# valeoai/NAF

Hardware: AMD Instinct MI355X
Metric: upsampled Mpixels/sec (NAF forward) (higher is better)
Workload: dtype bf16; 1 GPU; G1: 1x3x1024x1024 guidance, 1x768x64x64 features -> 1024x1024, window 7, per GPU; per_gpu_batch=1, global_batch=1, parallelism=batch-shard x1, scope=whole forward (conv stem + RoPE/pool + attention), weights=random-init NAF() defaults (dim 256, 4 heads), streams=2

## Files before the change

naf_amd/csrc/naf_api.hip:

```cpp
#include <stdarg.h>
#include <stdio.h>
#include <stdlib.h>
#include <string.h>

#include "naf_common.h"

static thread_local char g_err[512] = "";

void naf_set_error(const char* fmt, ...) {
    va_list ap;
    va_start(ap, fmt);
    vsnprintf(g_err, sizeof(g_err), fmt, ap);
    va_end(ap);
}

int naf_check_launch(const char* what) {
    const hipError_t e = hipGetLastError();
    if (e != hipSuccess) {
        naf_set_error("%s: %s", what, hipGetErrorString(e));
        return NAF_ERR_LAUNCH;
    }
    return NAF_OK;
}

// ... 599 lines not shown
    L.buf0 = off;  off = align256(off + px * 128 * 2);
    L.buf1 = off;  off = align256(off + px * 128 * 2);
    L.buf2 = off;  off = align256(off + px * 128 * 2);
    L.cat = off;   off = align256(off + px * 256 * 2);
    L.pooled = L.Ho != L.Hs || L.Wo != L.Ws;
    const size_t opx = (size_t)a->B * L.Ho * L.Wo;
    L.guide = L.pooled ? off : L.cat;
    if (L.pooled) off = align256(off + opx * 256 * 2);
    L.keys = off;  off = align256(off + (size_t)a->B * a->h * a->w * 256 * 2);
    L.vp = off;    off = align256(off + (size_t)a->B * a->h * a->w * a->C * 2);
    L.fused = fwd_rope_fusable(a);
    L.q = off;     off = align256(off + (L.fused ? 0 : opx * 256 * 2));
    L.idx_y = off; off = align256(off + (size_t)L.Ho * (a->ksize > 0 ? a->ksize : 1) * sizeof(int32_t));
    L.idx_x = off; off = align256(off + (size_t)L.Wo * (a->ksize > 0 ? a->ksize : 1) * sizeof(int32_t));
    L.total_one = off;
    L.buf3 = off;  off = align256(off + px * 128 * 2);
    L.total = off;
    return L;
}
int fwd_validate(const naf_forward_args* a) {
    NAF_REQUIRE(a != nullptr, "naf_forward: args is NULL");
    NAF_REQUIRE(a->image && a->features && a->out && a->tab_y && a->tab_x, "naf_forward: NULL tensor pointer");
    NAF_REQUIRE(a->B > 0 && a->H > 0 && a->W > 0 && a->h > 0 && a->w > 0 && a->C > 0 && a->heads > 0, "naf_forward: non-positive size");
    NAF_REQUIRE(a->nlayer >= 1 && a->nlayer <= NAF_MAX_STEM_LAYERS, "naf_forward: %d block layers (1..%d)", a->nlayer, NAF_MAX_STEM_LAYERS);
    NAF_REQUIRE(a->C % a->heads == 0, "naf_forward: %d feature channels not divisible by %d heads", a->C, a->heads);
    for (int br = 0; br < 2; ++br) {
        const naf_stem_branch& b = a->branch[br];
        NAF_REQUIRE(b.conv0_weight && b.conv0_bias, "naf_forward: branch %d: NULL conv0 parameters", br);
        NAF_REQUIRE((b.conv0_ksize == 1 || b.conv0_ksize == 3) && (b.ksize == 1 || b.ksize == 3), "naf_forward: branch %d: kernel sizes", br);
        for (int l = 0; l < a->nlayer; ++l)
            NAF_REQUIRE(b.gn_weight[l] && b.gn_bias[l] && b.conv_weight_packed[l] && b.conv_bias[l], "naf_forward: branch %d layer %d: NULL parameter", br, l);
    }
    return NAF_OK;
}
void fwd_xna_args(const naf_forward_args* a, const FwdLayout* L, bool fused, naf_xna_args* x) {
    char* ws = static_cast<char*>(a->workspace);
    const bool real = ws != nullptr && L != nullptr;
    const void* fake = reinterpret_cast<const void*>(0x100);
    const int Dv = a->C / a->heads;
    *x = naf_xna_args{};
    const int Ho = a->Ho > 0 ? a->Ho : a->H, Wo = a->Wo > 0 ? a->Wo : a->W;
    x->q = real ? ws + (fused ? L->guide : L->q) : fake;
    x->k_lr = real ? ws + L->keys : fake;
    x->v_lr = real ? ws + L->vp : fake;
    x->out = a->out;
    x->logits = a->logits;
    if (fused) {
        x->rope_tab_y = a->tab_y; x->rope_tab_x = a->tab_x;
        x->path = NAF_XNA_MFMA;
    } else {
        x->path = NAF_XNA_AUTO;
        x->idx_y = real ? reinterpret_cast<const int32_t*>(ws + L->idx_y) : static_cast<const int32_t*>(fake);
        x->idx_x = real ? reinterpret_cast<const int32_t*>(ws + L->idx_x) : static_cast<const int32_t*>(fake);
    }
    x->B = a->B; x->heads = a->heads; x->Ho = Ho; x->Wo = Wo; x->h = a->h; x->w = a->w;
    x->Dq = 256 / a->heads; x->Dv = Dv; x->ky = a->ksize; x->kx = a->ksize;
    x->out_dtype = a->out_dtype; x->scale = a->scale;
    const int64_t Dq = x->Dq;
    const int64_t qs[4] = {(int64_t)Ho * Wo * 256, Dq, (int64_t)Wo * 256, 256};
    const int64_t ks[4] = {(int64_t)a->h * a->w * 256, Dq, (int64_t)a->w * 256, 256};
    const int64_t vs[4] = {(int64_t)a->h * a->w * a->C, Dv, (int64_t)a->w * a->C, a->C};
    const int64_t os[4] = {(int64_t)Ho * Wo * a->C, Dv, (int64_t)Wo * a->C, a->C};
    for (int i = 0; i < 4; ++i) { x->q_stride[i] = qs[i]; x->k_stride[i] = ks[i]; x->v_stride[i] = vs[i]; x->o_stride[i] = os[i]; }
}
bool fwd_rope_fusable(const naf_forward_args* a) {
    if (a->heads_rope > 0 && a->heads_rope != a->heads) return false;
    if (a->heads <= 0 || a->C <= 0 || a->C % a->heads || 256 % a->heads) return false;
    naf_forward_args g = *a;
    g.workspace = nullptr;
    g.out = reinterpret_cast<void*>(0x100);
    g.tab_y = g.tab_x = reinterpret_cast<const float*>(0x100);
    naf_xna_args x;
    fwd_xna_args(&g, nullptr, true, &x);
    return xna_validate(&x) == NAF_OK && naf_xna_mfma_eligible(&x, nullptr, nullptr) && naf_xna_mfma_rope_ok(&x);
}
}

size_t naf_forward_workspace_bytes(const naf_forward_args* a) {
    if (a == nullptr || a->B <= 0 || a->H <= 0 || a->W <= 0 || a->h <= 0 || a->w <= 0 || a->C <= 0 || a->nlayer < 0) return 0;
    return fwd_layout(a).total;
}
size_t naf_forward_workspace_bytes_ex(const naf_forward_args* a, uint32_t flags) {
    if (a == nullptr || a->B <= 0 || a->H <= 0 || a->W <= 0 || a->h <= 0 || a->w <= 0 || a->C <= 0 || a->nlayer < 0) return 0;
    const FwdLayout L = fwd_layout(a);
    return (flags & NAF_FWD_ONE_STREAM) ? L.total_one : L.total;
}

int naf_forward_workspace_view(const naf_forward_args* a, int32_t which, size_t* offset, size_t* bytes) {
    NAF_REQUIRE(a != nullptr && offset != nullptr && bytes != nullptr, "naf_forward_workspace_view: NULL argument");
    NAF_REQUIRE(a->B > 0 && a->H > 0 && a->W > 0 && a->h > 0 && a->w > 0 && a->C > 0 && a->nlayer >= 0, "naf_forward_workspace_view: non-positive size");
    const FwdLayout L = fwd_layout(a);
    switch (which) {
        case NAF_FWD_BUF_GUIDANCE: *offset = L.guide; *bytes = (size_t)a->B * L.Ho * L.Wo * 256 * 2; return NAF_OK;
        case NAF_FWD_BUF_KEYS: *offset = L.keys; *bytes = (size_t)a->B * a->h * a->w * 256 * 2; return NAF_OK;
        case NAF_FWD_BUF_VALUES: *offset = L.vp; *bytes = (size_t)a->B * a->h * a->w * a->C * 2; return NAF_OK;
    }
    naf_set_error("naf_forward_workspace_view: unknown buffer %d", which);
    return NAF_ERR_INVALID;
}

int naf_forward_supported(const naf_forward_args* a) {
    const int rc = fwd_validate(a);
    if (rc != NAF_OK) return -rc;
    const int hr = a->heads_rope > 0 ? a->heads_rope : a->heads;
    if (256 % (4 * hr) != 0 || 256 % a->heads != 0 || (a->out_dtype != NAF_BF16 && a->out_dtype != NAF_F32)) return 0;
    const int Ho = a->Ho > 0 ? a->Ho : a->H, Wo = a->Wo > 0 ? a->Wo : a->W;
    if (a->H < 2 || a->W < 2 || Ho < a->h || Wo < a->w) return 0;
    {
        const FwdLayout Lq = fwd_layout(a);
        if (Lq.Hs < 2 || Lq.Ws < 2) return 0;
    }
    if (reinterpret_cast<uintptr_t>(a->out) % 16) return 0;
    if (fwd_rope_fusable(a)) return 1;
    naf_forward_args g = *a;
    g.workspace = nullptr;
    naf_xna_args x;
    fwd_xna_args(&g, nullptr, false, &x);
    return naf_xna_select(&x) > 0 ? 1 : 0;
}

namespace {
int fwd_streams(const naf_forward_args* a, uint32_t flags) {
    static const int knob = [] { const char* e = naf_knob("NAF_STEM_STREAMS"); return e ? atoi(e) : 0; }();
    if (fwd_sequential() || knob == 1 || (flags & NAF_FWD_ONE_STREAM)) return 1;
    if (knob == 2 || (flags & NAF_FWD_TWO_STREAMS)) return 2;
    const FwdLayout L = fwd_layout(a);
    const int k3 = a->branch[0].ksize == 3 ? 0 : (a->branch[1].ksize == 3 ? 1 : -1);
    if (k3 < 0 || a->branch[1 - k3].ksize == 3) return 2;
    int64_t nb = 0;
    const int seg_h = naf_stem_conv3_plan(a->B, L.Hs, L.Ws, false, &nb);
    const int ncu = naf_cu_count();
    return (nb <= ncu && nb > ncu - 4 && seg_h >= 12 && seg_h <= 40) ? 1 : 2;
}
}

int naf_forward_streams(const naf_forward_args* a, uint32_t flags) {
    const int sup = naf_forward_supported(a);
    if (sup <= 0) return sup;
    return fwd_streams(a, flags);
}

int naf_forward_aux_create(naf_forward_aux* out) {
    NAF_REQUIRE(out != nullptr, "naf_forward_aux_create: out is NULL");
    *out = naf_forward_aux{nullptr, nullptr, nullptr};
    hipStream_t st = nullptr;
    hipEvent_t fk = nullptr, jn = nullptr;
    const bool ok = hipStreamCreateWithFlags(&st, hipStreamNonBlocking) == hipSuccess &&
                    hipEventCreateWithFlags(&fk, hipEventDisableTiming) == hipSuccess &&
                    hipEventCreateWithFlags(&jn, hipEventDisableTiming) == hipSuccess;
    if (!ok) {
        (void)hipGetLastError();
        if (jn) (void)hipEventDestroy(jn);
        if (fk) (void)hipEventDestroy(fk);
        if (st) (void)hipStreamDestroy(st);
        naf_set_error("naf_forward_aux_create: cannot create a stream and two events on the current device");
        return NAF_ERR_LAUNCH;
    }
    out->stream = st; out->fork_event = fk; out->join_event = jn;
    return NAF_OK;
}

int naf_forward_aux_destroy(naf_forward_aux* aux) {
    NAF_REQUIRE(aux != nullptr, "naf_forward_aux_destroy: aux is NULL");
    bool ok = true;
    if (aux->join_event) ok &= hipEventDestroy(static_cast<hipEvent_t>(aux->join_event)) == hipSuccess;
    if (aux->fork_event) ok &= hipEventDestroy(static_cast<hipEvent_t>(aux->fork_event)) == hipSuccess;
    if (aux->stream) ok &= hipStreamDestroy(static_cast<hipStream_t>(aux->stream)) == hipSuccess;
    *aux = naf_forward_aux{nullptr, nullptr, nullptr};
    if (!ok) {
        (void)hipGetLastError();
        naf_set_error("naf_forward_aux_destroy: the HIP runtime refused a handle");
        return NAF_ERR_LAUNCH;
    }
    return NAF_OK;
}

int naf_forward(const naf_forward_args* a, naf_stream_t stream) { return naf_forward_ex(a, nullptr, 0u, stream); }

int naf_forward_ex(const naf_forward_args* a, const naf_forward_aux* aux, uint32_t flags, naf_stream_t stream) {
    const int sup = naf_forward_supported(a);
    if (sup < 0) return -sup;
    if (sup == 0) {
        naf_set_error("naf_forward: unsupported configuration (needs a head count dividing 64, output >= feature grid, kernel_size * "
                      "floor(ratio) <= output extent, 16-byte aligned output); compose the individual entry points instead");
        return NAF_ERR_UNSUPPORTED;
    }
    const FwdLayout L = fwd_layout(a);
    NAF_REQUIRE((flags & NAF_FWD_ONE_STREAM) == 0 || (flags & NAF_FWD_TWO_STREAMS) == 0, "naf_forward_ex: NAF_FWD_ONE_STREAM and NAF_FWD_TWO_STREAMS are exclusive");
    const bool may_fork = aux != nullptr && aux->stream != nullptr && (flags & NAF_FWD_ONE_STREAM) == 0;
    const size_t ws_need = may_fork ? L.total : L.total_one;
    NAF_REQUIRE(a->workspace != nullptr && a->workspace_bytes >= ws_need, "naf_forward: workspace of %zu bytes needed, %zu given", ws_need, a->workspace_bytes);
    NAF_REQUIRE(reinterpret_cast<uintptr_t>(a->workspace) % 256 == 0, "naf_forward: workspace must be 256-byte aligned");
    hipStream_t s = static_cast<hipStream_t>(stream);
    char* ws = static_cast<char*>(a->workspace);
    double* stats = reinterpret_cast<double*>(ws + L.stats);
    const size_t stat_stride = (size_t)NAF_STATS_SLOTS * a->B * 16;
    const bool have_aux = aux != nullptr && aux->stream != nullptr;
    NAF_REQUIRE(!have_aux || (aux->fork_event != nullptr && aux->join_event != nullptr), "naf_forward_ex: aux->stream without fork_event / join_event");
    NAF_REQUIRE(!have_aux || aux->stream != stream, "naf_forward_ex: aux->stream must differ from the stream of the call");
    if (hipMemsetAsync(stats, 0, L.zeroed, s) != hipSuccess) {
        naf_set_error("naf_forward: hipMemsetAsync failed");
        return NAF_ERR_LAUNCH;
    }
    void* bufs[3] = {ws + L.buf0, ws + L.buf1, ws + L.buf2};
    char* cat = ws + L.cat;
    auto mark = [&](int i) -> bool {
        if (a->phase_events[i] == nullptr) return true;
        if (hipEventRecord(static_cast<hipEvent_t>(a->phase_events[i]), s) == hipSuccess) return true;
        naf_set_error("naf_forward: hipEventRecord(phase_events[%d]) failed", i);
        return false;
    };
    if (!mark(0)) return NAF_ERR_LAUNCH;
    const void* simg = a->image;
    int simg_dtype = a->image_dtype;
    int64_t simg_stride[4] = {a->image_stride[0], a->image_stride[1], a->image_stride[2], a->image_stride[3]};
    const int SH = L.Hs, SW = L.Ws;
    if (L.shrunk) {
        const int src = naf_preshrink_image(reinterpret_cast<float*>(ws + L.img), a->image, a->image_dtype, a->B, a->H, a->W, SH, SW, a->image_stride, stream);
        if (src != NAF_OK) return src;
        simg = ws + L.img;
        simg_dtype = NAF_F32;
        simg_stride[0] = (int64_t)3 * SH * SW; simg_stride[1] = (int64_t)SH * SW; simg_stride[2] = SW; simg_stride[3] = 1;
    }
    const int64_t dense[3] = {(int64_t)SH * SW * 128, (int64_t)SW * 128, 128};
    const int64_t cat_st[3] = {(int64_t)SH * SW * 256, (int64_t)SW * 256, 256};
    static const bool sequential = [] { const char* e = naf_knob("NAF_STEM_ORDER"); return e && atoi(e) == 0; }();
    naf_stem_conv0_args c0s[2];
    naf_stream_t lstream = stream;
    auto run_conv0 = [&](int br, void* y) -> int {
        const naf_stem_branch& b = a->branch[br];
        naf_stem_conv0_args& c0 = c0s[br];
        c0 = naf_stem_conv0_args{};
        c0.image = simg; c0.weight = b.conv0_weight; c0.bias = b.conv0_bias; c0.stats_out = stats + (size_t)br * (a->nlayer + 1) * stat_stride;
        c0.image_dtype = simg_dtype; c0.ksize = b.conv0_ksize; c0.B = a->B; c0.H = SH; c0.W = SW;
        for (int i = 0; i < 4; ++i) c0.image_stride[i] = simg_stride[i];
        c0.y = y;
        for (int i = 0; i < 3; ++i) c0.y_stride[i] = dense[i];
        c0.flags = (flags & NAF_FWD_CONV0_EXACT) ? NAF_CONV0_EXACT : 0;
        return naf_stem_conv0_fwd(&c0, lstream);
    };
    static const bool no_keys_fuse = [] { const char* e = naf_knob("NAF_KEYS_FUSE"); return e && atoi(e) == 0; }();
    const int hrope_ = a->heads_rope > 0 ? a->heads_rope : a->heads;
    naf_key_pool_args kps[2];
    bool keys_fused = !no_keys_fuse && L.fused && !L.pooled && hrope_ == 4 && SH == 16 * a->h && SW == 16 * a->w;
    for (int br = 0; br < 2 && keys_fused; ++br) {
        kps[br] = naf_key_pool_args{};
        kps[br].k_lr = ws + L.keys + (size_t)br * 128 * 2;
        kps[br].tab_y = a->tab_y; kps[br].tab_x = a->tab_x; kps[br].h = a->h; kps[br].w = a->w;
        kps[br].k_stride[0] = (int64_t)a->h * a->w * 256; kps[br].k_stride[1] = (int64_t)a->w * 256; kps[br].k_stride[2] = 256;
        naf_stem_conv_args c{};
        c.x = reinterpret_cast<const void*>(0x100); c.y = reinterpret_cast<void*>(0x100); c.w_packed = reinterpret_cast<const void*>(0x100);
        c.bias = c.gn_weight = c.gn_bias = reinterpret_cast<const float*>(0x100); c.stats_in = reinterpret_cast<const double*>(0x100);
        c.ksize = a->branch[br].ksize; c.B = a->B; c.H = SH; c.W = SW;
        for (int i = 0; i < 3; ++i) { c.x_stride[i] = dense[i]; c.y_stride[i] = cat_st[i]; }
        const bool recomputed = a->nlayer == 1 && a->branch[br].conv0_ksize == 1 && a->branch[br].ksize == 1;
        if (recomputed || naf_stem_conv_keys_supported(&c, &kps[br]) != 1) keys_fused = false;
    }
    auto run_layer = [&](int br, int l, const void* x, void* y) -> int {
        const naf_stem_branch& b = a->branch[br];
        double* st = stats + (size_t)br * (a->nlayer + 1) * stat_stride;
        const bool last = l == a->nlayer - 1;
        naf_stem_conv_args c{};
        c.x = x;
        c.first = x == nullptr ? &c0s[br] : nullptr;
        c.y = last ? static_cast<void*>(cat + (size_t)br * 128 * 2) : y;
        c.w_packed = b.conv_weight_packed[l]; c.bias = b.conv_bias[l];
        c.gn_weight = b.gn_weight[l]; c.gn_bias = b.gn_bias[l];
        c.stats_in = st + (size_t)l * stat_stride;
        c.stats_out = last ? nullptr : st + (size_t)(l + 1) * stat_stride;
        c.ksize = b.ksize; c.B = a->B; c.H = SH; c.W = SW; c.eps = a->gn_eps;
        for (int i = 0; i < 3; ++i) { c.x_stride[i] = dense[i]; c.y_stride[i] = last ? cat_st[i] : dense[i]; }
        if (last && keys_fused) return naf_stem_conv_keys_fwd(&c, &kps[br], lstream);
        return naf_stem_conv_fwd(&c, lstream);
    };
    const bool rec[2] = {a->branch[0].conv0_ksize == 1 && a->branch[0].ksize == 1, a->branch[1].conv0_ksize == 1 && a->branch[1].ksize == 1};
    bool values_packed = false;
    StreamJoin sj;
    if (have_aux && !sequential && fwd_streams(a, flags) == 2) {
        const hipStream_t axs = static_cast<hipStream_t>(aux->stream);
        const hipEvent_t ev_fork = static_cast<hipEvent_t>(aux->fork_event);
        sj.s = s; sj.aux = axs; sj.ev = static_cast<hipEvent_t>(aux->join_event);
        const int timed = a->nlayer > 1 ? 1 : 0;
        auto mark_on = [&](int i, hipStream_t st) -> bool {
            if (a->phase_events[i] == nullptr) return true;
            if (hipEventRecord(static_cast<hipEvent_t>(a->phase_events[i]), st) == hipSuccess) return true;
            naf_set_error("naf_forward: hipEventRecord(phase_events[%d]) failed", i);
            return false;
        };
        const int first = (a->branch[0].ksize <= a->branch[1].ksize) ? 0 : 1;
        void* pp[2][2] = {{ws + L.buf0, ws + L.buf1}, {ws + L.buf2, ws + L.buf3}};
        void* cur[2] = {nullptr, nullptr};
        if (hipEventRecord(ev_fork, s) != hipSuccess || hipStreamWaitEvent(axs, ev_fork, 0) != hipSuccess) {
            (void)hipGetLastError();
            naf_set_error("naf_forward: stream fork failed");
            return NAF_ERR_LAUNCH;
        }
        sj.armed = true;
        {
            const int prc = naf_pack_values(ws + L.vp, a->features, a->feat_dtype, a->B, a->C, a->h, a->w, a->feat_stride, static_cast<naf_stream_t>(axs));
            if (prc != NAF_OK) return prc;
            values_packed = true;
        }
        static const bool fork_late = [] { const char* e = naf_knob("NAF_STEM_FORK_EARLY"); return !(e && atoi(e) != 0); }();
        for (int k = 0; k < 2; ++k) {
            const int br = k == 0 ? first : 1 - first;
            static const bool moments_aux = [] { const char* e = naf_knob("NAF_STEM_MOMENTS_AUX"); return e && atoi(e) != 0; }();
            lstream = (k == 0 && (!fork_late || (rec[br] && moments_aux))) ? static_cast<naf_stream_t>(axs) : stream;
            cur[br] = rec[br] ? nullptr : pp[br][0];
            const int rc = run_conv0(br, cur[br]);
            lstream = stream;
            if (rc != NAF_OK) return rc;
        }
        if (!mark(1)) return NAF_ERR_LAUNCH;
        if (fork_late && (hipEventRecord(ev_fork, s) != hipSuccess || hipStreamWaitEvent(axs, ev_fork, 0) != hipSuccess)) {
            (void)hipGetLastError();
            naf_set_error("naf_forward: stream fork failed");
            return NAF_ERR_LAUNCH;
        }
        for (int l = 0; l < a->nlayer; ++l)
            for (int k = 0; k < 2; ++k) {
                const int br = k == 0 ? first : 1 - first;
                static const bool swap_streams = [] { const char* e = naf_knob("NAF_STEM_SWAP"); return e && atoi(e) != 0; }();
                lstream = ((k == 0) != swap_streams) ? static_cast<naf_stream_t>(axs) : stream;
                void* y = (l == a->nlayer - 1) ? nullptr : pp[br][cur[br] == pp[br][0] ? 1 : 0];
                if (l == timed && k == 1 && !mark_on(2, s)) return NAF_ERR_LAUNCH;
                const int rc = run_layer(br, l, cur[br], y);
                lstream = stream;
                if (rc != NAF_OK) return rc;
                cur[br] = y;
                if (l == timed && !mark_on(k == 0 ? 3 : 7, k == 0 ? axs : s)) return NAF_ERR_LAUNCH;
            }
        const int jrc = sj.join();
        if (jrc != NAF_OK) return jrc;
    } else if (!sequential) {
        const int first = (a->branch[0].ksize <= a->branch[1].ksize) ? 0 : 1;
        const int order[2] = {first, 1 - first};
        bool busy[3] = {false, false, false};
        void* cur[2] = {nullptr, nullptr};
        auto grab = [&]() -> void* {
            for (int i = 0; i < 3; ++i)
                if (!busy[i]) { busy[i] = true; return bufs[i]; }
            return nullptr;
        };
        auto release = [&](const void* p) { for (int i = 0; i < 3; ++i) if (bufs[i] == p) busy[i] = false; };
        for (int k = 0; k < 2; ++k) {
            const int br = order[k];
            cur[br] = rec[br] ? nullptr : grab();
            const int rc = run_conv0(br, cur[br]);
            if (rc != NAF_OK) return rc;
        }
        if (!mark(1)) return NAF_ERR_LAUNCH;
        const int timed = a->nlayer > 1 ? 1 : 0;
        for (int l = 0; l < a->nlayer; ++l) {
            if (l == timed && !mark(2)) return NAF_ERR_LAUNCH;
            for (int k = 0; k < 2; ++k) {
                const int br = order[k];
                const bool last = l == a->nlayer - 1;
                void* y = last ? nullptr : grab();
                const int rc = run_layer(br, l, cur[br], y);
                if (rc != NAF_OK) return rc;
                release(cur[br]);
                cur[br] = y;
                if (l == timed && !mark(k == 0 ? 3 : 7)) return NAF_ERR_LAUNCH;
            }
        }
    } else {
        for (int br = 0; br < 2; ++br) {
            int rc = run_conv0(br, rec[br] ? nullptr : bufs[0]);
            if (rc != NAF_OK) return rc;
            if (!mark(1 + 2 * br)) return NAF_ERR_LAUNCH;
            const void* cur = bufs[0];
            for (int l = 0; l < a->nlayer; ++l) {
                void* y = bufs[(l + 1) & 1];
                rc = run_layer(br, l, (rec[br] && l == 0) ? nullptr : cur, y);
                if (rc != NAF_OK) return rc;
                cur = y;
            }
            if (br == 0 && !mark(2)) return NAF_ERR_LAUNCH;
        }
    }
    if (L.pooled) {
        const int prc = naf_pool_guidance(ws + L.guide, cat, a->B, SH, SW, L.Ho, L.Wo, 256, stream);
        if (prc != NAF_OK) return prc;
    }
    if (!mark(4)) return NAF_ERR_LAUNCH;
    naf_rope_pool_args rp{};
    rp.x = ws + L.guide; rp.q = L.fused ? nullptr : static_cast<void*>(ws + L.q); rp.k_lr = ws + L.keys; rp.tab_y = a->tab_y; rp.tab_x = a->tab_x;
    const int hrope = a->heads_rope > 0 ? a->heads_rope : a->heads;
    rp.x_dtype = NAF_BF16; rp.B = a->B; rp.Cq = 256; rp.heads = hrope; rp.Ho = L.Ho; rp.Wo = L.Wo; rp.h = a->h; rp.w = a->w;
    const int64_t xs[4] = {(int64_t)L.Ho * L.Wo * 256, 1, (int64_t)L.Wo * 256, 256};
    const int64_t kst[4] = {(int64_t)a->h * a->w * 256, 256 / hrope, (int64_t)a->w * 256, 256};
    const int64_t qst[4] = {(int64_t)L.Ho * L.Wo * 256, 256 / hrope, (int64_t)L.Wo * 256, 256};
    for (int i = 0; i < 4; ++i) { rp.x_stride[i] = xs[i]; rp.q_stride[i] = L.fused ? 0 : qst[i]; rp.k_stride[i] = kst[i]; }
    int rc = keys_fused ? NAF_OK : naf_rope_pool_fwd(&rp, stream);
    if (rc != NAF_OK) return rc;
    if (!values_packed) rc = naf_pack_values(ws + L.vp, a->features, a->feat_dtype, a->B, a->C, a->h, a->w, a->feat_stride, stream);
    if (rc != NAF_OK) return rc;
    naf_xna_args x;
    fwd_xna_args(a, &L, L.fused, &x);
    if (!L.fused && naf_xna_select(&x) != NAF_XNA_MFMA) {
        rc = naf_axis_index_table_device(reinterpret_cast<int32_t*>(ws + L.idx_y), L.Ho, a->h, a->ksize, stream);
        if (rc == NAF_OK) rc = naf_axis_index_table_device(reinterpret_cast<int32_t*>(ws + L.idx_x), L.Wo, a->w, a->ksize, stream);
        if (rc != NAF_OK) return rc;
    }
    if (!mark(5)) return NAF_ERR_LAUNCH;
    if (a->events[0] && hipEventRecord(static_cast<hipEvent_t>(a->events[0]), s) != hipSuccess) {
        naf_set_error("naf_forward: hipEventRecord failed");
        return NAF_ERR_LAUNCH;
    }
    {
        const int sel = naf_xna_select(&x);
        if (sel < 0) return -sel;
        if (sel == NAF_XNA_MFMA) {
            const float scale = x.scale > 0.f ? x.scale : 1.0f / sqrtf((float)x.Dq);
            rc = naf_launch_xna_mfma(&x, scale, s, reinterpret_cast<uint32_t*>(ws + L.steal));
        } else {
            rc = naf_xna_fwd(&x, stream);
        }
    }
    if (rc != NAF_OK) return rc;
    if (a->events[1] && hipEventRecord(static_cast<hipEvent_t>(a->events[1]), s) != hipSuccess) {
        naf_set_error("naf_forward: hipEventRecord failed");
        return NAF_ERR_LAUNCH;
    }
    if (!mark(6)) return NAF_ERR_LAUNCH;
    return NAF_OK;
}

}
```

naf_amd/csrc/stem_conv1x1.hip:

```cpp
#include <type_traits>

#include "naf_common.h"

struct StemConv1Params {
    const bf16_t* x;
    bf16_t* y;
    const bf16_t* w;
    const float* bias;
    const float* gamma;
    const float* beta;
    const double* stats_in;
    double* stats_out;
    int32_t B, H, W;
    int32_t groups_per_image;
    int32_t groups_per_block;
    float eps;
    int64_t xs[3], ys[3];
    const void* img;
    const float* w0;
    const float* b0;
    int64_t ibs;
    int32_t is[4];
    bf16_t* kout;
    const float* tab_y;
    const float* tab_x;
    int64_t kst[3];
    int32_t cw;
    int32_t ncell;
    int32_t cells_per_block;
};

namespace {
constexpr int C1 = 128, WROW = C1 + 8, OROW1 = C1 + 8;
#ifndef NAF_C1X1_NW
#define NAF_C1X1_NW 4
#endif
#ifndef NAF_C1_ABL
#define NAF_C1_ABL 0
#endif
constexpr int NW1 = NAF_C1X1_NW;
typedef float f32x16_t __attribute__((ext_vector_type(16)));
constexpr float kLog2e = 1.4426950408889634f;
}

#ifdef NAF_C1_TIMING
__device__ unsigned long long g_c1_tim[4096 * 8];
#define C1_T(i) do { const unsigned long long now_ = __builtin_amdgcn_s_memtime(); tacc[i] += now_ - tlast; tlast = now_; } while (0)
#else
#define C1_T(i) do { } while (0)
#endif

template <bool IMG, typename T, bool DENSE, bool PLAIN = false, bool POOL = false>
__global__ __launch_bounds__(NW1 * 64, (NW1 <= 4 ? 2 : 1)) void stem_conv1x1_kernel(const StemConv1Params p) {
    static_assert(!(IMG && PLAIN), "the recomputed-conv0 input exists for the forward layer only");
    static_assert(!POOL || (DENSE && !IMG && !PLAIN), "key pooling: dense forward layer reading its input from memory");
#ifdef NAF_C1_TIMING
    unsigned long long tacc[8] = {0, 0, 0, 0, 0, 0, 0, 0}, tlast = __builtin_amdgcn_s_memtime();
#endif
    extern __shared__ __attribute__((aligned(16))) unsigned char smem[];
    bf16_t* wl = reinterpret_cast<bf16_t*>(smem);
    bf16_t* ot = wl + C1 * WROW;
    float* cvec = reinterpret_cast<float*>(ot + NW1 * 32 * OROW1);

    const int tid = threadIdx.x, lane = tid & 63;
    const int wave = __builtin_amdgcn_readfirstlane(tid >> 6);
    const int n32 = lane & 31, half = lane >> 5;
    const int b = blockIdx.y;

    const int gbase = POOL ? blockIdx.x * p.cells_per_block : blockIdx.x * p.groups_per_block;
    const int ngroups = POOL ? min(p.ncell, gbase + p.cells_per_block) : min(p.groups_per_image, gbase + p.groups_per_block);
    const int gstride = NW1;
    const int npx = p.H * p.W;
    bf16_t* otw = ot + wave * 32 * OROW1;

    const int chk = lane & 15, psub = lane >> 4;
    const bool xdense = DENSE || p.xs[1] == (int64_t)p.W * p.xs[2], ydense = DENSE || p.ys[1] == (int64_t)p.W * p.ys[2];
    const bf16_t* xbase = p.x + b * p.xs[0] + chk * 8;
    const uint32_t lane_x = (uint32_t)(psub * (int)p.xs[2] + chk * 8) * 2u, lane_y = (uint32_t)(psub * (int)p.ys[2] + chk * 8) * 2u;
    const int nfull = npx >> 5;
    auto pool_group_off = [&](int cell, int gi, const int64_t (&st)[3]) __attribute__((always_inline)) {
        const int cc = cell < ngroups ? cell : ngroups - 1;
        const int cy = cc / p.cw, cx = cc - cy * p.cw;
        return (int64_t)(cy * 16 + 2 * gi) * st[1] + (int64_t)cx * 16 * st[2];
    };
    auto load_group = [&](int g, u32x4_t (&raw)[8], int gi = 0) __attribute__((always_inline)) {
        if constexpr (POOL) {
            const char* xg = reinterpret_cast<const char*>(p.x + b * p.xs[0] + pool_group_off(g, gi, p.xs));
            uint32_t lx = lane_x;
            asm volatile("" : "+v"(lx));
#pragma unroll
            for (int it = 0; it < 8; ++it)
                raw[it] = *reinterpret_cast<const u32x4_t*>(xg + (uint32_t)(lx + (uint32_t)(((it >> 2) * (int)p.xs[1] + (it & 3) * 4 * (int)p.xs[2]) * 2)));
            return;
        }
        const int gc = g < ngroups ? g : ngroups - 1;
        if (DENSE || (xdense && gc < nfull)) {
            const char* xg = reinterpret_cast<const char*>(p.x + b * p.xs[0] + (int64_t)gc * 32 * p.xs[2]);
            uint32_t lx = lane_x;
            asm volatile("" : "+v"(lx));
#pragma unroll
            for (int it = 0; it < 8; ++it) raw[it] = *reinterpret_cast<const u32x4_t*>(xg + (uint32_t)(lx + (uint32_t)(it * 8 * (int)p.xs[2])));
            return;
        }
        if constexpr (!DENSE) {
#pragma unroll
        for (int it = 0; it < 8; ++it) {
            const int n = min(gc * 32 + it * 4 + psub, npx - 1);
            int64_t off;
            if (xdense) {
                off = (int64_t)n * p.xs[2];
            } else {
                const int yy = n / p.W, xx = n - yy * p.W;
                off = (int64_t)yy * p.xs[1] + (int64_t)xx * p.xs[2];
            }
            raw[it] = *reinterpret_cast<const u32x4_t*>(xbase + off);
        }
        }
    };
    constexpr int WCH = C1 * (C1 / 8), WIT = (WCH + NW1 * 64 - 1) / (NW1 * 64);
    u32x4_t wst[WIT];
#pragma unroll
    for (int i = 0; i < WIT; ++i) {
        const int ci = min(tid + i * NW1 * 64, WCH - 1);
        wst[i] = *reinterpret_cast<const u32x4_t*>(p.w + (ci >> 4) * C1 + (ci & 15) * 8);
    }
    u32x4_t raw[8];
    if constexpr (!IMG) load_group(gbase + wave, raw);
#pragma unroll
    for (int i = 0; i < WIT; ++i) {
        const int ci = tid + i * NW1 * 64;
        if (WCH % (NW1 * 64) == 0 || ci < WCH) *reinterpret_cast<u32x4_t*>(wl + (ci >> 4) * WROW + (ci & 15) * 8) = wst[i];
    }
    if (tid < C1) {
        const int c = tid, g = c >> 4;
        if constexpr (PLAIN) {
            cvec[c] = p.bias ? p.bias[c] : 0.f;
        } else {
            const double n = (double)p.H * (double)p.W * 16.0;
            double s1, s2;
            naf_gn_sums(p.stats_in, p.B, b, g, s1, s2);
            const double mean = s1 / n;
            double var = s2 / n - mean * mean;
            var = var > 0.0 ? var : 0.0;
            const float rstd = (float)(1.0 / sqrt(var + (double)p.eps));
            const float gmm = p.gamma[c];
            cvec[c] = p.bias[c];
            cvec[C1 + c] = gmm * rstd * kLog2e;
            cvec[2 * C1 + c] = (p.beta[c] - (float)mean * gmm * rstd) * kLog2e;
            if constexpr (IMG) cvec[3 * C1 + c] = p.b0[c];
        }
    }
    __syncthreads();

    float ga[8], gb[8];
#pragma unroll
    for (int e = 0; e < 8; ++e) {
        ga[e] = cvec[C1 + chk * 8 + e];
        gb[e] = cvec[2 * C1 + chk * 8 + e];
    }

    f32x2_t s1p[8], s2p[8];
#pragma unroll
    for (int g = 0; g < 8; ++g) s1p[g] = s2p[g] = f32x2_t{0.f, 0.f};

    float w0r[4][2];
    const T* ib = nullptr;
    if constexpr (IMG) {
        ib = reinterpret_cast<const T*>(p.img) + (int64_t)b * p.ibs;
#pragma unroll
        for (int m = 0; m < 4; ++m)
#pragma unroll
            for (int ks = 0; ks < 2; ++ks) {
                const int k = 2 * ks + half;
                w0r[m][ks] = (k < 3) ? p.w0[(32 * m + n32) * 3 + k] : 0.f;
            }
    }
    auto load_taps = [&](int g, float (&sv)[2]) __attribute__((always_inline)) {
        const int gc = g < ngroups ? g : ngroups - 1;
        const int n = min(gc * 32 + n32, npx - 1);
        const int yy = n / p.W, xx = n - yy * p.W;
        const int o = yy * p.is[2] + xx * p.is[3];
        sv[0] = (float)ib[o + half * p.is[1]];
        sv[1] = (float)ib[o + 2 * p.is[1]];
    };

    float sv[2] = {0.f, 0.f};
    int g = gbase + wave;
    int gi = 0;
    f32x4_t pacc[8];
    float ptab[16];
    bf16x8_t pax;
    const int pG = lane >> 4, pli = lane & 15;
    if constexpr (POOL) {
#pragma unroll
        for (int j = 0; j < 8; ++j) pacc[j] = f32x4_t{0.f, 0.f, 0.f, 0.f};
#pragma unroll
        for (int i = 0; i < 16; ++i) ptab[i] = 0.f;
#pragma unroll
        for (int i = 0; i < 8; ++i) pax[i] = (bf16_t)((8 * (pG & 1) + i == pli) ? 1.0f : 0.0f);
    }
    if constexpr (IMG) load_taps(g, sv);
    if constexpr (IMG) asm volatile("; conv1x1 first group landed" ::"v"(sv[0]), "v"(sv[1]));
    else asm volatile("; conv1x1 first group landed" ::"v"(raw[0]), "v"(raw[1]), "v"(raw[2]), "v"(raw[3]), "v"(raw[4]), "v"(raw[5]), "v"(raw[6]), "v"(raw[7]));
    C1_T(0);
    for (; g < ngroups; g += (POOL ? 0 : gstride)) {
        const int n0 = g * 32;
#ifdef NAF_C1_TIMING
        if constexpr (!IMG) {
            asm volatile("s_waitcnt vmcnt(8)" ::: "memory");
            C1_T(1);
        }
#endif
        const float* cv = cvec;

        f32x16_t acc[4];
#pragma unroll
        for (int m = 0; m < 4; ++m)
#pragma unroll
            for (int j = 0; j < 4; ++j) {
                const f32x4_t bj = *reinterpret_cast<const f32x4_t*>(cv + 32 * m + 8 * j + 4 * half);
#pragma unroll
                for (int i = 0; i < 4; ++i) acc[m][j * 4 + i] = bj[i];
            }
        if constexpr (IMG) {
#pragma unroll
            for (int mp = 0; mp < 2; ++mp) {
                f32x16_t a0[2];
#pragma unroll
                for (int q = 0; q < 2; ++q) {
#pragma unroll
                    for (int r = 0; r < 16; ++r) a0[q][r] = 0.f;
#pragma unroll
                    for (int ks = 0; ks < 2; ++ks) a0[q] = __builtin_amdgcn_mfma_f32_32x32x2f32(w0r[2 * mp + q][ks], sv[ks], a0[q], 0, 0, 0);
                }
#pragma unroll
                for (int q = 0; q < 2; ++q) {
                    const int m = 2 * mp + q;
#pragma unroll
                    for (int j = 0; j < 4; ++j) {
                        const int c0 = 32 * m + 8 * j + 4 * half;
                        const f32x4_t bj = *reinterpret_cast<const f32x4_t*>(cv + 3 * C1 + c0);
                        const f32x4_t gaj = *reinterpret_cast<const f32x4_t*>(cv + C1 + c0);
                        const f32x4_t gbj = *reinterpret_cast<const f32x4_t*>(cv + 2 * C1 + c0);
                        bf16x4_t o;
#pragma unroll
                        for (int e = 0; e < 2; ++e) {
                            const f32x2_t v = f32x2_t{a0[q][j * 4 + 2 * e], a0[q][j * 4 + 2 * e + 1]} + f32x2_t{bj[2 * e], bj[2 * e + 1]};
                            bf16x2_t xb;
                            xb[0] = (bf16_t)v[0];
                            xb[1] = (bf16_t)v[1];
                            const f32x2_t x = {(float)xb[0], (float)xb[1]};
                            const f32x2_t y = x * f32x2_t{gaj[2 * e], gaj[2 * e + 1]} + f32x2_t{gbj[2 * e], gbj[2 * e + 1]};
                            const f32x2_t u = f32x2_t{__builtin_amdgcn_exp2f(-y[0]), __builtin_amdgcn_exp2f(-y[1])} * kLog2e + kLog2e;
                            const f32x2_t r = y * f32x2_t{__builtin_amdgcn_rcpf(u[0]), __builtin_amdgcn_rcpf(u[1])};
                            o[2 * e] = (bf16_t)r[0];
                            o[2 * e + 1] = (bf16_t)r[1];
                        }
                        *reinterpret_cast<bf16x4_t*>(otw + n32 * OROW1 + c0) = o;
                    }
                }
            }
        } else {
#pragma unroll
        for (int it = 0; it < 8; ++it) {
            if constexpr (PLAIN || (NAF_C1_ABL & 1)) {
                *reinterpret_cast<u32x4_t*>(otw + (it * 4 + psub) * OROW1 + chk * 8) = raw[it];
                continue;
            }
            bf16x8_t o;
#pragma unroll
            for (int e = 0; e < 4; ++e) {
                const uint32_t w = raw[it][e];
                const f32x2_t x = {__uint_as_float(w << 16), __uint_as_float(w & 0xffff0000u)};
                const f32x2_t y = x * f32x2_t{ga[2 * e], ga[2 * e + 1]} + f32x2_t{gb[2 * e], gb[2 * e + 1]};
                const f32x2_t u = f32x2_t{__builtin_amdgcn_exp2f(-y[0]), __builtin_amdgcn_exp2f(-y[1])} * kLog2e + kLog2e;
                const f32x2_t r = y * f32x2_t{__builtin_amdgcn_rcpf(u[0]), __builtin_amdgcn_rcpf(u[1])};
                o[2 * e] = (bf16_t)r[0];
                o[2 * e + 1] = (bf16_t)r[1];
            }
            *reinterpret_cast<bf16x8_t*>(otw + (it * 4 + psub) * OROW1 + chk * 8) = o;
        }
        }
        C1_T(2);
        __builtin_amdgcn_sched_barrier(0);
        if constexpr (IMG) load_taps(g + gstride, sv);
        else if constexpr (POOL) {
            load_group(gi == 7 ? g + gstride : g, raw, (gi + 1) & 7);
            if (gi == 7) {
                const int cy = g / p.cw, cx = g - cy * p.cw;
                const float* ty = p.tab_y + (int64_t)(cy * 16 + 4 * pG) * 32 + pli;
                const float* tx = p.tab_x + (int64_t)(cx * 16 + 4 * pG) * 32 + pli;
#pragma unroll
                for (int i = 0; i < 4; ++i) {
                    ptab[i] = ty[i * 32];
                    ptab[4 + i] = ty[i * 32 + 16];
                    ptab[8 + i] = tx[i * 32];
                    ptab[12 + i] = tx[i * 32 + 16];
                }
            }
        }
        else if constexpr (!(NAF_C1_ABL & 16)) load_group(g + gstride, raw);
        __builtin_amdgcn_sched_barrier(0);
        {
            bf16x8_t bfr[2], war[2][4];
            auto frag = [&](int ks, int slot) __attribute__((always_inline)) {
                bfr[slot] = *reinterpret_cast<const bf16x8_t*>(otw + n32 * OROW1 + ks * 16 + half * 8);
#pragma unroll
                for (int m = 0; m < 4; ++m) war[slot][m] = *reinterpret_cast<const bf16x8_t*>(wl + (m * 32 + n32) * WROW + ks * 16 + half * 8);
            };
            frag(0, 0);
#pragma unroll
            for (int ks = 0; ks < 8; ++ks) {
                __builtin_amdgcn_sched_barrier(0);
                if (ks + 1 < 8) frag(ks + 1, (ks + 1) & 1);
                __builtin_amdgcn_sched_barrier(0);
#pragma unroll
                for (int m = 0; m < 4; ++m) {
                    if constexpr (!(NAF_C1_ABL & 2)) acc[m] = __builtin_amdgcn_mfma_f32_32x32x16_bf16(war[ks & 1][m], bfr[ks & 1], acc[m], 0, 0, 0);
                    else asm volatile("" ::"v"(war[ks & 1][m]), "v"(bfr[ks & 1]));
                }
            }
            __builtin_amdgcn_sched_barrier(0);
        }
#ifdef NAF_C1_TIMING
        asm volatile("" ::"v"(acc[0]), "v"(acc[1]), "v"(acc[2]), "v"(acc[3]));
        C1_T(3);
#endif
        const bool full = DENSE || g < nfull;
        auto epilogue = [&](auto fullc) __attribute__((always_inline)) {
            constexpr bool FULL = decltype(fullc)::value;
            const float vmask = (FULL || (n0 + n32) < npx) ? 1.0f : 0.0f;
#pragma unroll
            for (int m = 0; m < 4; ++m)
#pragma unroll
                for (int j = 0; j < 4; ++j) {
                    const f32x2_t v0 = f32x2_t{acc[m][j * 4], acc[m][j * 4 + 1]}, v1 = f32x2_t{acc[m][j * 4 + 2], acc[m][j * 4 + 3]};
                    bf16x4_t o;
                    o[0] = (bf16_t)v0[0]; o[1] = (bf16_t)v0[1]; o[2] = (bf16_t)v1[0]; o[3] = (bf16_t)v1[1];
                    const f32x2_t w0 = FULL ? v0 : v0 * vmask, w1 = FULL ? v1 : v1 * vmask;
                    if constexpr (!(NAF_C1_ABL & 4) && !POOL) {
                        s1p[m * 2 + (j >> 1)] += w0 + w1;
                        s2p[m * 2 + (j >> 1)] += w0 * w0 + w1 * w1;
                    }
                    *reinterpret_cast<bf16x4_t*>(otw + n32 * OROW1 + 32 * m + 8 * j + 4 * half) = o;
                }
            C1_T(4);
            bf16_t* yb = p.y + b * p.ys[0];
            if constexpr (POOL) {
                char* yg = reinterpret_cast<char*>(yb + pool_group_off(g, gi, p.ys));
                uint32_t ly = lane_y;
                asm volatile("" : "+v"(ly));
#pragma unroll
                for (int it = 0; it < 8; ++it) {
                    const u32x4_t v = *reinterpret_cast<const u32x4_t*>(otw + (it * 4 + psub) * OROW1 + chk * 8);
                    *reinterpret_cast<u32x4_t*>(yg + (uint32_t)(ly + (uint32_t)(((it >> 2) * (int)p.ys[1] + (it & 3) * 4 * (int)p.ys[2]) * 2))) = v;
                }
                return;
            }
            if (FULL && (DENSE || ydense)) {
                char* yg = reinterpret_cast<char*>(yb + (int64_t)g * 32 * p.ys[2]);
                uint32_t ly = lane_y;
                asm volatile("" : "+v"(ly));
#pragma unroll
                for (int it = 0; it < 8; ++it) {
                    const u32x4_t v = *reinterpret_cast<const u32x4_t*>(otw + (it * 4 + psub) * OROW1 + chk * 8);
                    if constexpr (!(NAF_C1_ABL & 8)) *reinterpret_cast<u32x4_t*>(yg + (int64_t)it * 8 * p.ys[2] + ly) = v;
                    else asm volatile("" ::"v"(v));
                }
                C1_T(5);
                return;
            }
            if constexpr (!(FULL && DENSE)) {
#pragma unroll
            for (int it = 0; it < 8; ++it) {
                const int pp = it * 4 + psub, ch = chk;
                const int n = n0 + pp;
                if (n < npx) {
                    int64_t off;
                    if (ydense) {
                        off = (int64_t)n * p.ys[2];
                    } else {
                        const int yy = n / p.W, xx = n - yy * p.W;
                        off = (int64_t)yy * p.ys[1] + (int64_t)xx * p.ys[2];
                    }
                    const u32x4_t v = *reinterpret_cast<const u32x4_t*>(otw + pp * OROW1 + ch * 8);
                    *reinterpret_cast<u32x4_t*>(yb + off + ch * 8) = v;
                }
            }
            }
        };
        if constexpr (DENSE) {
            epilogue(std::true_type{});
        } else {
            if (full) epilogue(std::true_type{});
            else epilogue(std::false_type{});
        }
        if constexpr (POOL) {
            bf16x8_t pay;
            {
                const bf16_t one = (bf16_t)(((2 * gi + (pG >> 1)) == pli) ? 1.0f : 0.0f);
#pragma unroll
                for (int i = 0; i < 8; ++i) pay[i] = one;
            }
            const bf16_t* tb = otw + (8 * pG + (pli >> 2)) * OROW1 + (pli & 3) * 4;
#pragma unroll
            for (int j = 0; j < 8; ++j) {
                const bf16x4_t lo = __builtin_amdgcn_ds_read_tr16_b64_v4bf16((NAF_LDS bf16x4_t*)(tb + 16 * j));
                const bf16x4_t hi = __builtin_amdgcn_ds_read_tr16_b64_v4bf16((NAF_LDS bf16x4_t*)(tb + 4 * OROW1 + 16 * j));
                const bf16x8_t bt = {lo[0], lo[1], lo[2], lo[3], hi[0], hi[1], hi[2], hi[3]};
                pacc[j] = __builtin_amdgcn_mfma_f32_16x16x32_bf16((j & 1) ? pax : pay, bt, pacc[j], 0, 0, 0);
            }
            if (gi == 7) {
                const int cy = g / p.cw, cx = g - cy * p.cw;
                bf16_t* kc = p.kout + b * p.kst[0] + (int64_t)cy * p.kst[1] + (int64_t)cx * p.kst[2];
#pragma unroll
                for (int hh = 0; hh < 2; ++hh) {
                    float o[4] = {0.f, 0.f, 0.f, 0.f};
#pragma unroll
                    for (int i = 0; i < 4; ++i) {
                        float r1, r2;
                        naf_rope_rotate(pacc[4 * hh][i], pacc[4 * hh + 2][i], ptab[i], ptab[4 + i], r1, r2);
                        o[0] += r1;
                        o[2] += r2;
                        naf_rope_rotate(pacc[4 * hh + 1][i], pacc[4 * hh + 3][i], ptab[8 + i], ptab[12 + i], r1, r2);
                        o[1] += r1;
                        o[3] += r2;
                    }
#pragma unroll
                    for (int q = 0; q < 4; ++q) {
                        o[q] += __shfl_xor(o[q], 16);
                        o[q] += __shfl_xor(o[q], 32);
                    }
                    const float v = pG == 0 ? o[0] : pG == 1 ? o[1] : pG == 2 ? o[2] : o[3];
                    kc[64 * hh + lane] = (bf16_t)(v * (1.0f / 256.0f));
                }
#pragma unroll
                for (int j = 0; j < 8; ++j) pacc[j] = f32x4_t{0.f, 0.f, 0.f, 0.f};
                gi = 0;
                g += gstride;
            } else {
                ++gi;
            }
        }
    }

    if constexpr (IMG) asm volatile("; conv1x1 loop drained" ::"v"(sv[0]), "v"(sv[1]));
    else asm volatile("; conv1x1 loop drained" ::"v"(raw[0]), "v"(raw[1]), "v"(raw[2]), "v"(raw[3]), "v"(raw[4]), "v"(raw[5]), "v"(raw[6]), "v"(raw[7]));
#ifdef NAF_C1_TIMING
    if (lane == 0 && blockIdx.x < 512)
        for (int i = 0; i < 8; ++i) g_c1_tim[(blockIdx.x * NW1 + wave) * 8 + i] = tacc[i];
#endif
    if (p.stats_out) {
        __syncthreads();
        float* red = reinterpret_cast<float*>(ot);
#pragma unroll
        for (int gq = 0; gq < 8; ++gq) {
            float a = s1p[gq][0] + s1p[gq][1], q = s2p[gq][0] + s2p[gq][1];
#pragma unroll
            for (int o = 32; o > 0; o >>= 1) {
                a += __shfl_xor(a, o);
                q += __shfl_xor(q, o);
            }
            if (lane == 0) {
                red[wave * 16 + gq] = a;
                red[wave * 16 + 8 + gq] = q;
            }
        }
        __syncthreads();
        if (tid < 16) {
            float a = 0.f;
#pragma unroll
            for (int wv = 0; wv < NW1; ++wv) a += red[wv * 16 + tid];
            atomicAdd(&naf_gn_slot(p.stats_out, p.B, b, blockIdx.x)[(tid & 7) * 2 + (tid >> 3)], (double)a);
        }
    }
}

int naf_stem_conv1x1_keys_ok(const naf_stem_conv_args* a, const naf_key_pool_args* kp) {
    return a->ksize == 1 && a->first == nullptr && a->stats_in != nullptr && a->stats_out == nullptr && (a->channels == 0 || a->channels == 128) &&
           a->H == 16 * kp->h && a->W == 16 * kp->w && a->x_stride[1] == (int64_t)a->W * a->x_stride[2] &&
           a->y_stride[1] == (int64_t)a->W * a->y_stride[2] && a->x_stride[1] * 2 < 0x7fffffffLL && a->y_stride[1] * 2 < 0x7fffffffLL;
}

int naf_launch_stem_conv1x1(const naf_stem_conv_args* a, hipStream_t s, const naf_key_pool_args* kp) {
    StemConv1Params p;
    p.x = static_cast<const bf16_t*>(a->x);
    p.y = static_cast<bf16_t*>(a->y);
    p.w = static_cast<const bf16_t*>(a->w_packed);
    p.bias = a->bias; p.gamma = a->gn_weight; p.beta = a->gn_bias;
    p.stats_in = a->stats_in; p.stats_out = a->stats_out;
    p.B = a->B; p.H = a->H; p.W = a->W; p.eps = a->eps;
    for (int i = 0; i < 3; ++i) { p.xs[i] = a->x_stride[i]; p.ys[i] = a->y_stride[i]; }
    p.groups_per_image = (int)(((int64_t)a->H * a->W + 31) / 32);
    const size_t lds = (size_t)(C1 * WROW + NW1 * 32 * OROW1) * 2 + 4 * C1 * sizeof(float);
    const int64_t slots = (int64_t)naf_cu_count() * (NW1 <= 4 ? 2 : 1) * NW1;
    const int64_t total = (int64_t)p.groups_per_image * a->B;
    const int64_t gpw = (total + slots - 1) / slots;
    static const int gpw_knob = [] { const char* e = naf_knob("NAF_C1X1_GPW"); return e ? atoi(e) : 0; }();
    const int64_t gpw_eff = gpw_knob > 0 ? gpw_knob : gpw;
    p.groups_per_block = (int32_t)(gpw_eff * NW1);
    int64_t nbx = (p.groups_per_image + p.groups_per_block - 1) / p.groups_per_block;
    if (nbx < 1) nbx = 1;
    if (a->B > 65535) {
        naf_set_error("naf_stem_conv_fwd: batch %d out of range", a->B);
        return NAF_ERR_INVALID;
    }
    p.img = nullptr; p.w0 = nullptr; p.b0 = nullptr; p.ibs = 0;
    for (int i = 0; i < 4; ++i) p.is[i] = 0;
    p.kout = nullptr; p.tab_y = p.tab_x = nullptr; p.cw = p.ncell = p.cells_per_block = 0;
    for (int i = 0; i < 3; ++i) p.kst[i] = 0;
    if (kp != nullptr) {
        if (!naf_stem_conv1x1_keys_ok(a, kp)) {
            naf_set_error("naf_stem_conv_keys_fwd: the 1x1 kernel needs 16 x 16 pixel cells, dense rows, stats_out == NULL and first == NULL");
            return NAF_ERR_UNSUPPORTED;
        }
        p.kout = static_cast<bf16_t*>(kp->k_lr); p.tab_y = kp->tab_y; p.tab_x = kp->tab_x;
        for (int i = 0; i < 3; ++i) p.kst[i] = kp->k_stride[i];
        p.cw = kp->w; p.ncell = kp->h * kp->w;
        const int64_t cpw = ((int64_t)p.ncell * a->B + slots - 1) / slots;
        p.cells_per_block = (int32_t)(cpw * NW1);
        nbx = (p.ncell + p.cells_per_block - 1) / p.cells_per_block;
    }
    int variant = 0;
    if (a->first != nullptr) {
        const naf_stem_conv0_args* f = a->first;
        const int64_t span = 2 * llabs(f->image_stride[1]) + (int64_t)(a->H - 1) * llabs(f->image_stride[2]) +
                             (int64_t)(a->W - 1) * llabs(f->image_stride[3]);
        if (span >= 0x7fffffffLL) {
            naf_set_error("naf_stem_conv_fwd: first: image too large for 32-bit tap offsets (span %lld elements)", (long long)span);
            return NAF_ERR_UNSUPPORTED;
        }
        p.img = f->image; p.w0 = f->weight; p.b0 = f->bias; p.ibs = f->image_stride[0];
        for (int i = 0; i < 4; ++i) p.is[i] = (int32_t)f->image_stride[i];
        variant = f->image_dtype == NAF_BF16 ? 2 : 1;
    }
    const dim3 grid((uint32_t)nbx, (uint32_t)a->B), blk(NW1 * 64);
    if (kp != nullptr) {
        auto kern = stem_conv1x1_kernel<false, float, true, false, true>;
        if (hipFuncSetAttribute(reinterpret_cast<const void*>(kern), hipFuncAttributeMaxDynamicSharedMemorySize, (int)lds) != hipSuccess) {
            naf_set_error("naf_stem_conv_keys_fwd: cannot reserve %zu bytes of LDS", (size_t)lds);
            return NAF_ERR_LAUNCH;
        }
        hipLaunchKernelGGL(kern, grid, blk, lds, s, p);
        return naf_check_launch("stem_conv1x1_kernel<keys>");
    }
#define NAF_LAUNCH_1X1(KERN)                                                                                              \
    do {                                                                                                                  \
        if (hipFuncSetAttribute(reinterpret_cast<const void*>(KERN), hipFuncAttributeMaxDynamicSharedMemorySize, (int)lds) != hipSuccess) { \
            naf_set_error("naf_stem_conv_fwd: cannot reserve %zu bytes of LDS", (size_t)lds);                             \
            return NAF_ERR_LAUNCH;                                                                                        \
        }                                                                                                                 \
        hipLaunchKernelGGL(KERN, grid, blk, lds, s, p);                                                                   \
    } while (0)
    const bool dense = (a->x_stride[1] == (int64_t)a->W * a->x_stride[2] || a->first != nullptr) &&
                       a->y_stride[1] == (int64_t)a->W * a->y_stride[2] && (((int64_t)a->H * a->W) % 32 == 0);
    if (a->stats_in == nullptr) {
        if (dense) NAF_LAUNCH_1X1((stem_conv1x1_kernel<false, float, true, true>));
        else NAF_LAUNCH_1X1((stem_conv1x1_kernel<false, float, false, true>));
    } else if (dense) {
        if (variant == 0) NAF_LAUNCH_1X1((stem_conv1x1_kernel<false, float, true>));
        else if (variant == 1) NAF_LAUNCH_1X1((stem_conv1x1_kernel<true, float, true>));
        else NAF_LAUNCH_1X1((stem_conv1x1_kernel<true, bf16_t, true>));
    } else {
        if (variant == 0) NAF_LAUNCH_1X1((stem_conv1x1_kernel<false, float, false>));
        else if (variant == 1) NAF_LAUNCH_1X1((stem_conv1x1_kernel<true, float, false>));
        else NAF_LAUNCH_1X1((stem_conv1x1_kernel<true, bf16_t, false>));
    }
#undef NAF_LAUNCH_1X1
    return naf_check_launch("stem_conv1x1_kernel");
}
```

Before: 562.3 Mpix/s.

## Recompute conv0 on VALU via LDS tap transpose and add late-moments scheduling knob

Replaces the recomputed 3-channel conv0 inside the fused 1x1 stem conv, which used fp32 32x32x2 MFMAs plus a separate bias/GELU path, with a VALU FMA computation. Pixel taps are transposed through a small per-wave LDS scratch so each lane holds the channel layout of the raw-input path, and the result feeds the existing normalize/activation loop. This removes duplicated epilogue code and cuts the MFMA work on a K=3 problem. It also adds a dense-image fast path for tap addressing, plus a knob (default off) that defers the moments-only conv0 launch until after the stream fork. The cost is extra LDS space and LDS traffic per group.

```diff
diff --git a/naf_amd/csrc/naf_api.hip b/naf_amd/csrc/naf_api.hip
--- a/naf_amd/csrc/naf_api.hip
+++ b/naf_amd/csrc/naf_api.hip
@@ -925,11 +925,17 @@
             values_packed = true;
         }
         static const bool fork_late = [] { const char* e = naf_knob("NAF_STEM_FORK_EARLY"); return !(e && atoi(e) != 0); }();
+        static const bool swap_streams = [] { const char* e = naf_knob("NAF_STEM_SWAP"); return e && atoi(e) != 0; }();
+        static const int moments_at = [] { const char* e = naf_knob("NAF_STEM_MOMENTS"); return e ? atoi(e) : 0; }();
+        bool moments_late[2] = {false, false};
         for (int k = 0; k < 2; ++k) {
             const int br = k == 0 ? first : 1 - first;
-            static const bool moments_aux = [] { const char* e = naf_knob("NAF_STEM_MOMENTS_AUX"); return e && atoi(e) != 0; }();
-            lstream = (k == 0 && (!fork_late || (rec[br] && moments_aux))) ? static_cast<naf_stream_t>(axs) : stream;
             cur[br] = rec[br] ? nullptr : pp[br][0];
+            if (fork_late && rec[br] && moments_at == 2) {
+                moments_late[br] = true;
+                continue;
+            }
+            lstream = (k == 0 && (!fork_late || (rec[br] && moments_at == 1))) ? static_cast<naf_stream_t>(axs) : stream;
             const int rc = run_conv0(br, cur[br]);
             lstream = stream;
             if (rc != NAF_OK) return rc;
@@ -940,10 +946,17 @@
             naf_set_error("naf_forward: stream fork failed");
             return NAF_ERR_LAUNCH;
         }
+        for (int k = 0; k < 2; ++k) {
+            const int br = k == 0 ? first : 1 - first;
+            if (!moments_late[br]) continue;
+            lstream = ((k == 0) != swap_streams) ? static_cast<naf_stream_t>(axs) : stream;
+            const int rc = run_conv0(br, nullptr);
+            lstream = stream;
+            if (rc != NAF_OK) return rc;
+        }
         for (int l = 0; l < a->nlayer; ++l)
             for (int k = 0; k < 2; ++k) {
                 const int br = k == 0 ? first : 1 - first;
-                static const bool swap_streams = [] { const char* e = naf_knob("NAF_STEM_SWAP"); return e && atoi(e) != 0; }();
                 lstream = ((k == 0) != swap_streams) ? static_cast<naf_stream_t>(axs) : stream;
                 void* y = (l == a->nlayer - 1) ? nullptr : pp[br][cur[br] == pp[br][0] ? 1 : 0];
                 if (l == timed && k == 1 && !mark_on(2, s)) return NAF_ERR_LAUNCH;
diff --git a/naf_amd/csrc/stem_conv1x1.hip b/naf_amd/csrc/stem_conv1x1.hip
--- a/naf_amd/csrc/stem_conv1x1.hip
+++ b/naf_amd/csrc/stem_conv1x1.hip
@@ -61,6 +61,7 @@
     bf16_t* wl = reinterpret_cast<bf16_t*>(smem);
     bf16_t* ot = wl + C1 * WROW;
     float* cvec = reinterpret_cast<float*>(ot + NW1 * 32 * OROW1);
+    float* tapl = cvec + 4 * C1;
 
     const int tid = threadIdx.x, lane = tid & 63;
     const int wave = __builtin_amdgcn_readfirstlane(tid >> 6);
@@ -147,7 +148,6 @@
             cvec[c] = p.bias[c];
             cvec[C1 + c] = gmm * rstd * kLog2e;
             cvec[2 * C1 + c] = (p.beta[c] - (float)mean * gmm * rstd) * kLog2e;
-            if constexpr (IMG) cvec[3 * C1 + c] = p.b0[c];
         }
     }
     __syncthreads();
@@ -163,25 +163,81 @@
 #pragma unroll
     for (int g = 0; g < 8; ++g) s1p[g] = s2p[g] = f32x2_t{0.f, 0.f};
 
-    float w0r[4][2];
+    f32x2_t w0p[3][4], b0p[4];
     const T* ib = nullptr;
+    float* tapw = tapl + wave * 96;
     if constexpr (IMG) {
         ib = reinterpret_cast<const T*>(p.img) + (int64_t)b * p.ibs;
 #pragma unroll
-        for (int m = 0; m < 4; ++m)
-#pragma unroll
-            for (int ks = 0; ks < 2; ++ks) {
-                const int k = 2 * ks + half;
-                w0r[m][ks] = (k < 3) ? p.w0[(32 * m + n32) * 3 + k] : 0.f;
-            }
-    }
+        for (int e = 0; e < 4; ++e) {
+            const int c = chk * 8 + 2 * e;
+#pragma unroll
+            for (int k = 0; k < 3; ++k) w0p[k][e] = f32x2_t{p.w0[c * 3 + k], p.w0[(c + 1) * 3 + k]};
+            b0p[e] = f32x2_t{p.b0[c], p.b0[c + 1]};
+        }
+    }
+    const bool idense = p.is[2] == p.W * p.is[3];
     auto load_taps = [&](int g, float (&sv)[2]) __attribute__((always_inline)) {
+        if constexpr (NAF_C1_ABL & 16) return;
         const int gc = g < ngroups ? g : ngroups - 1;
         const int n = min(gc * 32 + n32, npx - 1);
-        const int yy = n / p.W, xx = n - yy * p.W;
-        const int o = yy * p.is[2] + xx * p.is[3];
+        int o;
+        if (idense) {
+            o = n * p.is[3];
+        } else {
+            const int yy = n / p.W, xx = n - yy * p.W;
+            o = yy * p.is[2] + xx * p.is[3];
+        }
         sv[0] = (float)ib[o + half * p.is[1]];
         sv[1] = (float)ib[o + 2 * p.is[1]];
+    };
+    auto conv0_group = [&](const float (&sv)[2], u32x4_t (&raw)[8]) __attribute__((always_inline)) {
+        float tx[3][8];
+        if constexpr (NAF_C1_ABL & 64) {
+#pragma unroll
+            for (int it = 0; it < 8; ++it) { tx[0][it] = sv[0] + (float)it; tx[1][it] = sv[1] - (float)it; tx[2][it] = sv[0] * (float)(it + 1); }
+        } else {
+            const int wi = (n32 & 3) * 24 + (n32 >> 2);
+            tapw[wi + half * 8] = sv[0];
+            tapw[wi + 16] = sv[1];
+            asm volatile("" ::: "memory");
+#pragma unroll
+            for (int c = 0; c < 3; ++c) {
+                const f32x4_t lo = *reinterpret_cast<const f32x4_t*>(tapw + psub * 24 + c * 8), hi = *reinterpret_cast<const f32x4_t*>(tapw + psub * 24 + c * 8 + 4);
+#pragma unroll
+                for (int i = 0; i < 4; ++i) { tx[c][i] = lo[i]; tx[c][4 + i] = hi[i]; }
+            }
+            asm volatile("" ::: "memory");
+        }
+#pragma unroll
+        for (int it = 0; it < 8; ++it)
+#pragma unroll
+            for (int eh = 0; eh < 4; eh += 2) {
+                f32x2_t v[2];
+                if constexpr (NAF_C1_ABL & 32) {
+#pragma unroll
+                    for (int e = 0; e < 2; ++e) v[e] = f32x2_t{tx[0][it], tx[1][it]} + b0p[eh + e];
+                } else {
+                    const f32x2_t x0 = {tx[0][it], tx[0][it]}, x1 = {tx[1][it], tx[1][it]}, x2 = {tx[2][it], tx[2][it]};
+#pragma unroll
+                    for (int e = 0; e < 2; ++e) v[e] = __builtin_elementwise_fma(w0p[0][eh + e], x0, f32x2_t{0.f, 0.f});
+#pragma unroll
+                    for (int e = 0; e < 2; ++e) v[e] = __builtin_elementwise_fma(w0p[1][eh + e], x1, v[e]);
+#pragma unroll
+                    for (int e = 0; e < 2; ++e) v[e] = __builtin_elementwise_fma(w0p[2][eh + e], x2, v[e]);
+#pragma unroll
+                    for (int e = 0; e < 2; ++e) v[e] = __builtin_elementwise_fma(f32x2_t{0.f, 0.f}, x2, v[e]);
+#pragma unroll
+                    for (int e = 0; e < 2; ++e) v[e] = v[e] + b0p[eh + e];
+                }
+#pragma unroll
+                for (int e = 0; e < 2; ++e) {
+                    bf16x2_t xb;
+                    xb[0] = (bf16_t)v[e][0];
+                    xb[1] = (bf16_t)v[e][1];
+                    raw[it][eh + e] = __builtin_bit_cast(uint32_t, xb);
+                }
+            }
     };
 
     float sv[2] = {0.f, 0.f};
@@ -206,10 +262,8 @@
     for (; g < ngroups; g += (POOL ? 0 : gstride)) {
         const int n0 = g * 32;
 #ifdef NAF_C1_TIMING
-        if constexpr (!IMG) {
-            asm volatile("s_waitcnt vmcnt(8)" ::: "memory");
-            C1_T(1);
-        }
+        asm volatile("s_waitcnt vmcnt(8)" ::: "memory");
+        C1_T(1);
 #endif
         const float* cv = cvec;
 
@@ -223,44 +277,13 @@
                 for (int i = 0; i < 4; ++i) acc[m][j * 4 + i] = bj[i];
             }
         if constexpr (IMG) {
-#pragma unroll
-            for (int mp = 0; mp < 2; ++mp) {
-                f32x16_t a0[2];
-#pragma unroll
-                for (int q = 0; q < 2; ++q) {
-#pragma unroll
-                    for (int r = 0; r < 16; ++r) a0[q][r] = 0.f;
-#pragma unroll
-                    for (int ks = 0; ks < 2; ++ks) a0[q] = __builtin_amdgcn_mfma_f32_32x32x2f32(w0r[2 * mp + q][ks], sv[ks], a0[q], 0, 0, 0);
-                }
-#pragma unroll
-                for (int q = 0; q < 2; ++q) {
-                    const int m = 2 * mp + q;
-#pragma unroll
-                    for (int j = 0; j < 4; ++j) {
-                        const int c0 = 32 * m + 8 * j + 4 * half;
-                        const f32x4_t bj = *reinterpret_cast<const f32x4_t*>(cv + 3 * C1 + c0);
-                        const f32x4_t gaj = *reinterpret_cast<const f32x4_t*>(cv + C1 + c0);
-                        const f32x4_t gbj = *reinterpret_cast<const f32x4_t*>(cv + 2 * C1 + c0);
-                        bf16x4_t o;
-#pragma unroll
-                        for (int e = 0; e < 2; ++e) {
-                            const f32x2_t v = f32x2_t{a0[q][j * 4 + 2 * e], a0[q][j * 4 + 2 * e + 1]} + f32x2_t{bj[2 * e], bj[2 * e + 1]};
-                            bf16x2_t xb;
-                            xb[0] = (bf16_t)v[0];
-                            xb[1] = (bf16_t)v[1];
-                            const f32x2_t x = {(float)xb[0], (float)xb[1]};
-                            const f32x2_t y = x * f32x2_t{gaj[2 * e], gaj[2 * e + 1]} + f32x2_t{gbj[2 * e], gbj[2 * e + 1]};
-                            const f32x2_t u = f32x2_t{__builtin_amdgcn_exp2f(-y[0]), __builtin_amdgcn_exp2f(-y[1])} * kLog2e + kLog2e;
-                            const f32x2_t r = y * f32x2_t{__builtin_amdgcn_rcpf(u[0]), __builtin_amdgcn_rcpf(u[1])};
-                            o[2 * e] = (bf16_t)r[0];
-                            o[2 * e + 1] = (bf16_t)r[1];
-                        }
-                        *reinterpret_cast<bf16x4_t*>(otw + n32 * OROW1 + c0) = o;
-                    }
-                }
-            }
-        } else {
+            conv0_group(sv, raw);
+#ifdef NAF_C1_TIMING
+            asm volatile("" ::"v"(raw[0]), "v"(raw[1]), "v"(raw[2]), "v"(raw[3]), "v"(raw[4]), "v"(raw[5]), "v"(raw[6]), "v"(raw[7]));
+            C1_T(6);
+#endif
+        }
+        {
 #pragma unroll
         for (int it = 0; it < 8; ++it) {
             if constexpr (PLAIN || (NAF_C1_ABL & 1)) {
@@ -492,7 +515,7 @@
     p.B = a->B; p.H = a->H; p.W = a->W; p.eps = a->eps;
     for (int i = 0; i < 3; ++i) { p.xs[i] = a->x_stride[i]; p.ys[i] = a->y_stride[i]; }
     p.groups_per_image = (int)(((int64_t)a->H * a->W + 31) / 32);
-    const size_t lds = (size_t)(C1 * WROW + NW1 * 32 * OROW1) * 2 + 4 * C1 * sizeof(float);
+    const size_t lds = (size_t)(C1 * WROW + NW1 * 32 * OROW1) * 2 + 4 * C1 * sizeof(float) + (a->first != nullptr ? NW1 * 96 * sizeof(float) : 0);
     const int64_t slots = (int64_t)naf_cu_count() * (NW1 <= 4 ? 2 : 1) * NW1;
     const int64_t total = (int64_t)p.groups_per_image * a->B;
     const int64_t gpw = (total + slots - 1) / slots;
```

Result: no change. 562.5 Mpix/s, median of 6 (+0.0%).
